# moritzmeister/hops-examples

Hardware: AMD Instinct MI355X
Metric: images/sec MNIST CNN + steps/sec Chicago-taxi DNN at 1/2/4/8 MI355X (higher is better)
Workload: dtype bf16; 1 GPU; model=MNIST CNN (experiment.mirrored model, 1394282 params), Adadelta(1.0), global_batch=32, per_gpu_batch=32, parallelism=dp1, engine=PersistentMnistStep, hipgraph=False, steps_per_execution=32, warmup_steps_run=5

## Files before the change

csrc/ops/bindings.cpp:

```cpp
#include <pybind11/pybind11.h>
#include <pybind11/stl.h>

#include <algorithm>
#include <memory>
#include <stdexcept>
#include <string>
#include <tuple>
#include <utility>
#include <vector>

#if defined(HOPSX_DEBUG) && HOPSX_DEBUG
#define HOPSX_DEBUG_BUILD 1
#else
#define HOPSX_DEBUG_BUILD 0
#endif

#include "ops_api.h"
extern "C" int hopsx_mnist_persist_occupancy(int dp);
extern "C" void hopsx_mnist_persist_reload_knobs();
extern "C" int hopsx_pad_cin(const float* w, long R, int C, int cp, float* out, void* out16, hipStream_t st);
extern "C" int hopsx_unpad_cin_add(float* gpad, long R, int C, int cp, float* tgt, hipStream_t st);

namespace py = pybind11;
extern "C" void hopsx_mlp_head_debug(void* p);
// ... 69 lines not shown
                      P<float>(arowsum), P<unsigned>(tickets), S(st));
  });
  m.def("conv2d_fwd", [](u x, u w, std::vector<int> g, int epi, u out, u bias, int act, u colsum, float xscale,
                         float xshift, u st) {
    return hopsx_conv2d_fwd(P<void>(x), P<void>(w), g.data(), epi, P<void>(out), P<float>(bias), act,
                            P<float>(colsum), xscale, xshift, S(st));
  });
  m.def("conv2d_fwd_res", [](u x, u w, std::vector<int> g, u out, u bias, int act, u residual, u st) {
    return hopsx_conv2d_fwd_res(P<void>(x), P<void>(w), g.data(), P<void>(out), P<float>(bias), act,
                                P<void>(residual), S(st));
  });
  m.def("conv2d_fwd_res_path", [](std::vector<int> g) { return hopsx_conv2d_fwd_res_path(g.data()); });
  m.def("conv2d_dgrad", [](u dy, u w, std::vector<int> g, u dx, u yprev, int act, u colsum, u y, int yact, u addend,
                           u st) {
    return hopsx_conv2d_dgrad(P<void>(dy), P<void>(w), g.data(), P<void>(dx), P<void>(yprev), act, P<float>(colsum),
                              P<void>(y), yact, P<void>(addend), S(st));
  });
  m.def("widedeep_slots", [](std::vector<long> iv, u out, long n) {
    return hopsx_widedeep_slots(iv.data(), (int)iv.size(), P<int>(out), n);
  });
  m.def("taxi_step2_ok", [](std::vector<long> iv, long rows) { return hopsx_taxi_step2_ok(iv.data(), (int)iv.size(), rows); });
  m.def("taxi_step2_xgeom", []() {
    std::vector<long> g(4);
    hopsx_taxi_step2_xgeom(g.data());
    return g;
  });
  m.def("taxi_step2", [](std::vector<uint64_t> p, std::vector<long> iv, std::vector<float> fv, long rows, u st) {
    return hopsx_taxi_step2(p.data(), (int)p.size(), iv.data(), (int)iv.size(), fv.data(), (int)fv.size(), rows, S(st));
  });
  def_arg_slots<true>(m, "taxi_step2", [](const ArgSlots& a, hipStream_t st) {
    return hopsx_taxi_step2(a.p.data(), (int)a.p.size(), a.iv.data(), (int)a.iv.size(), a.fv.data(), (int)a.fv.size(),
                            a.extra, st);
  });
  m.def("widedeep_step_lds", [](std::vector<long> iv) { return hopsx_widedeep_step_lds(iv.data(), (int)iv.size()); });
  m.def("set_deterministic", [](int on) {
    int e = 0;
#define X(tag) \
  if (!e) e = hopsx_det_set_##tag(on);
    HOPSX_DET_TUS(X)
#undef X
    return e;
  });
  m.attr("DEBUG") = HOPSX_DEBUG_BUILD;
  m.def("dbg_read", []() {
    static const std::pair<const char*, int (*)(unsigned*)> tus[] = {
#define X(tag) {#tag, hopsx_dbg_read_##tag},
        HOPSX_DBG_TUS(X)
#undef X
    };
    std::vector<std::tuple<std::string, unsigned, unsigned, unsigned, unsigned>> out;
    for (const auto& t : tus) {
      unsigned v[4] = {0u, 0u, 0u, 0u};
      const int e = t.second(v);
      if (e) throw std::runtime_error(std::string("hopsx dbg_read: hip error ") + std::to_string(e));
      if (v[0]) out.emplace_back(t.first, v[0], v[1], v[2], v[3]);
    }
    return out;
  });
  m.def("det_lost", []() {
    unsigned n = 0;
#define X(tag) n += hopsx_det_lost_##tag();
    HOPSX_DET_TUS(X)
#undef X
    return n;
  });
  m.def("mnist_persist", [](std::vector<uint64_t> p, std::vector<long> iv, std::vector<float> fv, u st) {
    return hopsx_mnist_persist(p.data(), (int)p.size(), iv.data(), (int)iv.size(), fv.data(), (int)fv.size(),
                               S(st));
  });
  def_arg_slots<false>(m, "mnist_persist", [](const ArgSlots& a, hipStream_t st) {
    return hopsx_mnist_persist(a.p.data(), (int)a.p.size(), a.iv.data(), (int)a.iv.size(), a.fv.data(),
                               (int)a.fv.size(), st);
  });
  m.def("mnist_eval", [](std::vector<uint64_t> p, std::vector<long> iv, std::vector<float> fv, u st) {
    return hopsx_mnist_eval(p.data(), (int)p.size(), iv.data(), (int)iv.size(), fv.data(), (int)fv.size(), S(st));
  });
  m.def("mnist_eval_tile", []() { return hopsx_mnist_eval_tile(); });
  m.def("taxi_eval", [](std::vector<uint64_t> p, std::vector<long> iv, u st) {
    return hopsx_taxi_eval(p.data(), (int)p.size(), iv.data(), (int)iv.size(), S(st));
  });
  m.def("taxi_eval_bins", []() { return hopsx_taxi_eval_bins(); });
  m.def("mnist_persist_reload_knobs", []() { hopsx_mnist_persist_reload_knobs(); });
  m.def("mnist_persist_occupancy", [](int dp) { return hopsx_mnist_persist_occupancy(dp); });
  m.def("pad_cin", [](u w, long R, int C, int cp, u out, u out16, u st) {
    return hopsx_pad_cin(P<float>(w), R, C, cp, P<float>(out), P<void>(out16), S(st));
  });
  m.def("unpad_cin_add", [](u g, long R, int C, int cp, u tgt, u st) {
    return hopsx_unpad_cin_add(P<float>(g), R, C, cp, P<float>(tgt), S(st));
  });
  m.def("mnist_persist_geom", []() {
    std::vector<long> g(24);
    hopsx_mnist_persist_geom(g.data());
    return g;
  });
  m.def("widedeep_step", [](std::vector<uint64_t> p, std::vector<long> iv, std::vector<float> fv, u st) {
    return hopsx_widedeep_step(p.data(), (int)p.size(), iv.data(), (int)iv.size(), fv.data(), (int)fv.size(),
                               S(st));
  });
  m.def("conv2d_fwd_pool_ok", [](std::vector<int> g, int act, int pk) { return hopsx_conv_fwd_pool_ok(g.data(), act, pk); });
  m.def("conv2d_fwd_pool", [](u x, u w, std::vector<int> g, u out, u am, u bias, int act, float p, u rng,
                              unsigned salt, int pk, u st) {
    return hopsx_conv2d_fwd_pool(P<void>(x), P<void>(w), g.data(), P<void>(out), P<void>(am), P<float>(bias), act, p,
                                 P<unsigned long long>(rng), salt, pk, S(st));
  });
  m.def("conv2d_fwd_pool_in_ok", [](std::vector<int> g0, std::vector<int> g, int act) {
    return hopsx_conv_fwd_pool_in_ok(g0.data(), g.data(), act);
  });
  m.def("conv2d_fwd_pool_in", [](u x0, float xscale, float xshift, u w0, u b0, int act0, std::vector<int> g0, u y1,
                                 u w, std::vector<int> g, u out, u am, u bias, int act, float p, u rng, unsigned salt,
                                 u st) {
    return hopsx_conv2d_fwd_pool_in(P<void>(x0), xscale, xshift, P<void>(w0), P<float>(b0), act0, g0.data(),
                                    P<void>(y1), P<void>(w), g.data(), P<void>(out), P<void>(am), P<float>(bias), act,
                                    p, P<unsigned long long>(rng), salt, S(st));
  });
  m.def("conv2d_dgrad_fused_wgrad_ok", [](std::vector<int> g, std::vector<int> g0) {
    return hopsx_conv_dgrad_fused_wgrad_ok(g.data(), g0.data());
  });
  m.def("conv2d_dgrad_fused_wgrad", [](u dy, u w, std::vector<int> g, u yprev, int act, u colsum, u y, int yact,
                                       std::vector<int> g0, u x0, float xscale, float xshift, u dw0, u st) {
    return hopsx_conv2d_dgrad_mfma_ex(P<void>(dy), P<void>(w), g.data(), nullptr, P<void>(yprev), act,
                                      P<float>(colsum), P<void>(y), yact, g0.data(), P<void>(x0), xscale, xshift,
                                      P<float>(dw0), S(st));
  });
  m.def("wgrad_debug_times", [](int n) {
    std::vector<unsigned long long> v((size_t)n);
    hopsx_wgrad_debug_times(v.data(), n);
    return v;
  });
  m.def("head_ce_ok", [](int C, int KD) { return hopsx_head_ce_ok(C, KD); });
  m.def("head_ce", [](int kind, u logits, int lf32, u target, int B, int C, int KD, float gs, u h, u w, u dw, u db,
                      u dh, u loss, u correct, u bias, u lout, float dp, u drng, unsigned dsalt, u st) {
    return hopsx_head_ce(kind, P<void>(logits), lf32, P<void>(target), B, C, KD, gs, P<void>(h), P<void>(w),
                         P<float>(dw), P<float>(db), P<void>(dh), P<float>(loss), P<int>(correct), P<float>(bias),
                         P<void>(lout), dp, P<unsigned long long>(drng), dsalt, S(st));
  });
  m.def("mlp_head_lds", [](int C, int N1) { return hopsx_mlp_head_lds(C, N1); });
  m.def("mlp_head_debug", [](u p) { hopsx_mlp_head_debug(P<void>(p)); });
  m.def("graph_upload", [](u exec, u st) {
    return (int)hipGraphUpload(reinterpret_cast<hipGraphExec_t>(exec), S(st));
  });
  m.def("mlp_head", [](u x, u w1, u b1, int act1, u y, u ws, u arrive, int B, int K, int N1, int kind, u target,
                       int C, float gs, u w2, u b2, u dw2, u db2, u dh, u loss, u correct, u lout, int lf32, float dp,
                       u drng, unsigned dsalt, u st) {
    return hopsx_mlp_head(P<void>(x), P<void>(w1), P<float>(b1), act1, P<void>(y), P<float>(ws), P<unsigned>(arrive),
                          B, K, N1, kind, P<void>(target), C, gs, P<void>(w2), P<float>(b2), P<float>(dw2),
                          P<float>(db2), P<void>(dh), P<float>(loss), P<int>(correct), P<void>(lout), lf32, dp,
                          P<unsigned long long>(drng), dsalt, S(st));
  });
  m.def("zero", [](u p, long bytes, u st) { return hopsx_zero(P<void>(p), bytes, S(st)); });
  m.def("nonfinite", [](u x, long n, int is_bf16, u out, u st) {
    return hopsx_nonfinite(P<void>(x), n, is_bf16, P<unsigned>(out), S(st));
  });
  m.def("linear_bwd_pair", [](u dy, u w, u x, u dx, u yprev, int act_prev, u colsum, u ay, int aact, u dw, u db,
                              int M, int N, int K, std::vector<int> pool, u pam, u px, u prng, unsigned psalt,
                              float pp, int dw_store, u st) {
    return hopsx_linear_bwd_pair(P<void>(dy), P<void>(w), P<void>(x), P<void>(dx), P<void>(yprev), act_prev,
                                 P<float>(colsum), P<void>(ay), aact, P<float>(dw), P<float>(db), M, N, K,
                                 pool.empty() ? nullptr : pool.data(), P<unsigned char>(pam), P<void>(px),
                                 P<unsigned long long>(prng), psalt, pp, dw_store, S(st));
  });
  m.def("conv2d_bwd_pair", [](u dy, u w, std::vector<int> g, u dx, u yprev, int act, u colsum, u y, int yact,
                              std::vector<int> g0, u x0, float xscale, float xshift, u dw0, u x, u dw, u db, u add,
                              u bnz, u bnmean, u bnrstd, u bnacc, u st) {
    return hopsx_conv2d_bwd_pair(P<void>(dy), P<void>(w), g.data(), P<void>(dx), P<void>(yprev), act,
                                 P<float>(colsum), P<void>(y), yact, g0.empty() ? nullptr : g0.data(), P<void>(x0),
                                 xscale, xshift, P<float>(dw0), P<void>(x), P<float>(dw), P<float>(db), P<void>(add),
// ... 186 lines not shown
```

csrc/ops/common.h:

```cpp
#pragma once
#include <hip/hip_runtime.h>
#include <stdint.h>

#define HOPSX_WAVE 64

typedef uint16_t bf16_raw;
typedef short bf16x8 __attribute__((ext_vector_type(8)));
typedef short bf16x4 __attribute__((ext_vector_type(4)));
typedef float f32x4 __attribute__((ext_vector_type(4)));

__device__ __forceinline__ bf16x8 zero_unless(bf16x8 v, bool keep) {
  const short m = keep ? (short)-1 : (short)0;
  return v & (bf16x8){m, m, m, m, m, m, m, m};
}
typedef __attribute__((address_space(3))) bf16x4* lds_v4_ptr;

__device__ __forceinline__ float bf2f(uint16_t v) { return __uint_as_float(((uint32_t)v) << 16); }

__device__ __forceinline__ uint16_t f2bf(float f) {
  uint32_t u = __float_as_uint(f);
  if ((u & 0x7fffffffu) > 0x7f800000u) return 0x7fc0;
  u += 0x7fffu + ((u >> 16) & 1u);
  return (uint16_t)(u >> 16);
}

__device__ __forceinline__ float wave_sum(float v) {
#pragma unroll
  for (int o = 32; o > 0; o >>= 1) v += __shfl_xor(v, o, 64);
  return v;
}
__device__ __forceinline__ float wave_max(float v) {
#pragma unroll
  for (int o = 32; o > 0; o >>= 1) v = fmaxf(v, __shfl_xor(v, o, 64));
  return v;
}

template <int R>
__device__ __forceinline__ float dpp_ror(float v) {
  return __builtin_bit_cast(float, __builtin_amdgcn_update_dpp(0, __builtin_bit_cast(int, v), 0x120 + R, 0xF, 0xF, false));
}
template <int CW>
__device__ __forceinline__ float row_fold(float v) {
  if constexpr (CW <= 1) v += dpp_ror<1>(v);
  if constexpr (CW <= 2) v += dpp_ror<2>(v);
  if constexpr (CW <= 4) v += dpp_ror<4>(v);
  if constexpr (CW <= 8) v += dpp_ror<8>(v);
  return v;
}

constexpr int kArriveWords = 9 * 32;
constexpr int HOPSX_BN_NREP = 8;
__device__ inline bool grid_arrive_last(unsigned* arrive) {
  const unsigned G = gridDim.x;
  const unsigned shard = blockIdx.x & 7u;
  const unsigned members = (G - shard + 7u) / 8u;
  unsigned* sw = arrive + 32u * (shard + 1u);
  if (atomicAdd(sw, 1u) != members - 1u) return false;
  atomicExch(sw, 0u);
  const unsigned shards = G < 8u ? G : 8u;
  if (atomicAdd(arrive, 1u) != shards - 1u) return false;
  atomicExch(arrive, 0u);
  return true;
}

__device__ __forceinline__ int xcd_remap(int bid, int nwg) {
  if (nwg <= 8) return bid;
  const int xcd = bid & 7, q = nwg >> 3, r = nwg & 7;
  const int base = (xcd < r) ? xcd * (q + 1) : r * (q + 1) + (xcd - r) * q;
  return base + (bid >> 3);
}

__device__ __forceinline__ uint32_t mix32(uint32_t x) {
  x ^= x >> 16;
  x *= 0x7feb352du;
  x ^= x >> 15;
  x *= 0x846ca68bu;
  x ^= x >> 16;
  return x;
}
__device__ __forceinline__ uint32_t hash_u32(uint64_t seed, uint64_t idx) {
  const uint32_t ka = (uint32_t)seed ^ (uint32_t)(idx >> 32) * 0x9E3779B9u;
  const uint32_t kb = (uint32_t)(seed >> 32);
  return mix32(mix32((uint32_t)idx ^ ka) + kb);
}
__device__ __forceinline__ float uniform01(uint64_t seed, uint64_t idx) {
  return (hash_u32(seed, idx) & 0xFFFFFF) * (1.0f / 16777216.0f);
}

__device__ __forceinline__ uint64_t drop_key(const unsigned long long* rng, unsigned salt) {
  return (uint64_t)rng[0] ^ ((uint64_t)salt * 0xD1B54A32D192ED03ull) ^ ((uint64_t)rng[1] * 0x8CB92BA72F3D8DD7ull);
}

enum Act : int { ACT_NONE = 0, ACT_RELU = 1, ACT_SIGMOID = 2, ACT_TANH = 3 };

__device__ __forceinline__ float apply_act(float v, int act) {
  switch (act) {
    case ACT_RELU: return v > 0.f ? v : 0.f;
    case ACT_SIGMOID: return 1.f / (1.f + __expf(-v));
    case ACT_TANH: return tanhf(v);
    default: return v;
  }
}
__device__ __forceinline__ float act_grad_from_out(float y, int act) {
  switch (act) {
    case ACT_RELU: return y > 0.f ? 1.f : 0.f;
    case ACT_SIGMOID: return y * (1.f - y);
    case ACT_TANH: return 1.f - y * y;
    default: return 1.f;
  }
}

#define HOPSX_CHECK_LAUNCH() (void)hipGetLastError()

#include <cstdlib>
#include <cstring>
static inline bool hopsx_disabled(const char* name) {
  const char* env = std::getenv("HOPSX_DISABLE");
  return env && *env && std::strstr(env, name) != nullptr;
}
static inline long hopsx_env_int(const char* name, long dflt) {
  const char* e = std::getenv(name);
  return e && *e ? std::atol(e) : dflt;
}

static inline bool hopsx_deterministic() {
  static const bool on = [] {
    const char* e = std::getenv("HOPSX_DETERMINISTIC");
    return e && *e == '1';
  }();
// ... 71 lines not shown
```

csrc/ops/mnist_persist.hip:

```cpp
#include "common.h"
#include "mnist_cnn.h"
#include "optim_core.h"
#include "wg_prims.h"

namespace mnistp {
using namespace wgp;
using namespace mnist_cnn;

constexpr int B = 32;
constexpr int NCONV = C2 * 128 + C2 + C1 * 4 + C1;
constexpr int OFF_B2 = C2 * 128, OFF_W1 = OFF_B2 + C2, OFF_B1 = OFF_W1 + C1 * 4;
constexpr int SLICE = 64, NSLICE = (NCONV + SLICE - 1) / SLICE;
constexpr int NRED = 19;
constexpr int NKC = (NPOS + NRED - 1) / NRED;
constexpr int NQ = SLICE / 4;
constexpr int NHEAD = B;
constexpr int GRID = NPOS + NHEAD;
constexpr int PAY = 272;
constexpr int PAY_DH = 0, PAY_H = 128, PAY_DL = 256, PAY_LOSS = 268, PAY_COR = 269;
constexpr int FL_A = 0, FL_B = 256, FL_C = 512, FL_D = 768, FL_WORDS = 1024;
constexpr int FL_EPOCH = FL_WORDS - 2;
constexpr int D_F32 = OFF_B2 * 2;
constexpr int D_BYTES = D_F32 + (NCONV - OFF_B2) * 4;
constexpr int TGB_N = NHEAD * (HID / 2);
constexpr int TG_WORDS = 2 * 2 * TGB_N;
static_assert(FL_WORDS % 2 == 0 && TGB_N % 256 == 0, "granules are 8-B aligned; every thread owns TGB_N / 256");
constexpr int HAND_FILL_C = 1 << 16;
constexpr int HAND_FILL_KEEP = 1 << 17;
constexpr int HAND_FMAX_SHIFT = 20;
constexpr int FCH = 4, NFCH = 32 / FCH;
static_assert(32 % FCH == 0 && NFCH <= 15, "whole chunks; the cap fits its 4 bits of Args::hand");

constexpr int DHS = row_stride(HID), DCS = row_stride(4 * B);
static_assert(DHS == 136 && DCS == 136, "strides the kernel was tuned with");

constexpr int L_W1 = 0;
constexpr int L_W2 = L_W1 + HID * W1S * 2;
constexpr int L_CW1 = L_W2 + C2 * W2S * 2;
constexpr int L_CB1 = L_CW1 + C1 * 4 * 4;
constexpr int L_CB2 = L_CB1 + C1 * 4;
constexpr int L_XIN = L_CB2 + C2 * 4;
constexpr int L_C1 = L_XIN + B * 16 * 4;
constexpr int L_POOL = L_C1 + B * 9 * C1S * 2;
constexpr int L_AM = L_POOL + B * PLS * 2;
constexpr int L_DH = L_AM + B * C2;
constexpr int L_DC2 = L_DH + B * DHS * 2;
constexpr int L_STG = L_DC2 + C2 * DCS * 2;
constexpr int L_RED = L_STG + NCONV * 4;
constexpr int L_SL = L_RED + NRED * SLICE * 4;
constexpr int L_KEEP = L_SL + 3 * 64 * 4;
constexpr int LDS_BYTES = L_KEEP + B * C2;

constexpr int H_W2 = 0;
constexpr int H_B2 = H_W2 + 3 * NCLS * HID * 4;
constexpr int H_B1 = H_B2 + 3 * 16 * 4;
constexpr int H_RED = H_B1 + 3 * HID * 4;
constexpr int H_H = H_RED + 8 * HID * 4;
constexpr int H_LOG = H_H + HID * 4;
constexpr int H_PAY = H_LOG + 16 * 4;
constexpr int H_ALL = H_PAY + PAY * 4;
constexpr int H_END = H_ALL + NHEAD * PAY * 4;
constexpr int H_DHS = H_END;
static_assert(H_DHS + B * DHS * 2 <= LDS_BYTES, "head LDS map must fit the position map");

constexpr int XMAX = 8;
constexpr long XS_POOL = (long)NPOS * 4 * 64 * 16;
constexpr long XS_DHT = 8L * 64 * 16;
constexpr int NFC2 = NCLS * HID + HID + NCLS, NFC2P = 1424;
constexpr long XS_FC2 = NFC2P * 4;
constexpr long XS_CONV = (long)NSLICE * SLICE * 4;
constexpr long XO_POOL = 0, XO_DHT = XO_POOL + 2L * XMAX * XS_POOL, XO_FC2 = XO_DHT + 2L * XMAX * XS_DHT,
               XO_CONV = XO_FC2 + 2L * XMAX * XS_FC2, X_BYTES = XO_CONV + 2L * XMAX * XS_CONV;
constexpr int XF_POOL = 0, XF_H = XMAX * NPOS, XF_CONV = XF_H + XMAX, XF_WORDS = XF_CONV + XMAX * NSLICE;
static_assert(NFC2 <= NFC2P && NFC2P % 4 == 0 && X_BYTES < 0x7fffffffL, "exchange geometry");
static_assert(LDS_BYTES <= 160 * 1024, "one workgroup per CU: 160 KiB LDS");
static_assert(L_RED + NRED * SLICE * 4 <= L_SL && 2 * 32 * 5 * 4 <= NRED * SLICE * 4, "reduce scratch");
static_assert(SLICE * 4 % 128 == 0 && NCONV * 4 % 128 == 0, "a slice row is whole 128-byte lines of an aligned slabC row");
static_assert(OFF_B2 % SLICE == 0 && D_F32 % 128 == 0 && D_BYTES % 128 == 0, "no slice straddles the bf16 / fp32 parts of D");
static_assert(NSLICE * SLICE >= NCONV && NSLICE <= NPOS && SLICE == 64, "slice geometry: one wave updates a slice");
static_assert(NQ == 16 && NRED > 16 && NRED - 16 <= 3 && 5 * NKC <= 64 && 2 * NKC <= 32 && NRED * (NKC - 1) < NPOS,
              "gather geometry: at most 5 groups' flags per wave, one per lane; both items' rows in one pend mask");

struct Args {
  float* master;
  bf16_raw* shadow;
  float* s1;
  float* s2;
  long off[8];
  const unsigned char* xs;
  const long long* ys;
  long nbatch;
  long long* cursor;
  unsigned long long* rng;
  float* step_dev;
  const float* hp_dev;
  float* slabA;
  float* slabB;
  float* slabC;
  float* slabD;
  unsigned* flags;
  unsigned* err;
  float* out;
  unsigned long long* dbg;
  OptHP hp;
  float drop_p, xscale, xshift;
  unsigned salt;
  int nsteps;
  int acquire;
  long long tmo;
  long long tmo0;
  int pollw, stagger;
  int pollw_a, pollw_b, pollw_c, pollw_d;
  int head1w;
  int hand;
  float inv_gb;
  int world, rank;
  int loopback;
  int xfence;
  long long* xstep;
  unsigned char* xbuf[XMAX];
  unsigned* xflag[XMAX];
};


__device__ __forceinline__ int xslot(const Args& a, int peer) { return a.loopback ? peer : a.rank; }

__device__ __forceinline__ bool wait_all(const unsigned* flags, int n, unsigned epoch, unsigned* err, unsigned code,
                                      int acquire, int* s_ok, long long tmo, int pollw = 1, int stagger = 0,
                                      int poll1 = 0) {
  if (pollw <= 1) {
    if (threadIdx.x < 64) {
      const int lane = threadIdx.x;
      int good = 1;
      const long long t0 = wall_clock64();
      for (unsigned spins = 0;; ++spins) {
        int ok = 1;
        unsigned e = poll1 ? flag_load(err) : 0u;
        for (int k = lane; k < n; k += 64) ok &= flag_load(flags + k) == epoch;
        if (__all(ok)) break;
        if (!poll1) e = flag_load(err);
        if (__builtin_amdgcn_readfirstlane(e) != 0u) {
          good = 0;
          break;
        }
        if ((spins & 15u) == 15u && wall_clock64() - t0 > tmo) {
          if (lane == 0) atomicCAS(err, 0u, code);
          good = 0;
          break;
        }
        __builtin_amdgcn_s_sleep(1);
      }
      if (acquire && good) __builtin_amdgcn_fence(__ATOMIC_ACQUIRE, "agent");
      drain();
      if (lane == 0) *s_ok = good;
    }
    __syncthreads();
    const int g = *s_ok;
    return g != 0;
  }
  volatile int* gen = s_ok + 1;
  const int wave = threadIdx.x >> 6;
  if (wave < pollw) {
    const int lane = threadIdx.x & 63;
    int good = 1;
    for (int d = 0; d < wave * stagger && __builtin_amdgcn_readfirstlane(*gen) != (int)code; ++d)
      __builtin_amdgcn_s_sleep(1);
    const long long t0 = wall_clock64();
    for (unsigned spins = 0;; ++spins) {
      if (__builtin_amdgcn_readfirstlane(*gen) == (int)code) break;
      int ok = 1;
      unsigned e = poll1 ? flag_load(err) : 0u;
      for (int k = lane; k < n; k += 64) ok &= flag_load(flags + k) == epoch;
      if (__all(ok)) {
        if (lane == 0) {
          s_ok[0] = 1;
          *gen = (int)code;
        }
        break;
      }
      if (!poll1) e = flag_load(err);
      if (__builtin_amdgcn_readfirstlane(e) != 0u) good = 0;
      if ((spins & 15u) == 15u && wall_clock64() - t0 > tmo) {
        if (lane == 0) atomicCAS(err, 0u, code);
        good = 0;
      }
      if (!good) {
        if (lane == 0) {
          s_ok[0] = 0;
          *gen = (int)code;
        }
        break;
      }
      __builtin_amdgcn_s_sleep(1);
    }
    if (acquire) __builtin_amdgcn_fence(__ATOMIC_ACQUIRE, "agent");
    drain();
  }
// ... 862 lines not shown
    for (int j = 0; j < 4; ++j)
#pragma unroll
      for (int r = 0; r < 4; ++r) {
        const int n = (2 * w + ii) * 16 + fq * 4 + r, co = j * 16 + fr;
        const long ai = a.off[4] + (long)n * KIN + p * C2 + co;
        a.master[ai] = wm[ii][j][r];
        a.s1[ai] = g1[ii][j][r];
        a.s2[ai] = g2[ii][j][r];
        a.shadow[ai] = f2bf_hw(wm[ii][j][r]);
      }
  if (owner && tid < SLICE) {
    const int e = p * SLICE + tid;
    if (e < NCONV) {
      const long ci = conv_idx(a, e);
      a.master[ci] = SLm[tid];
      a.s1[ci] = SL1[tid];
      a.s2[ci] = SL2[tid];
      a.shadow[ci] = f2bf_hw(SLm[tid]);
    }
  }
  stamp(a, a.nsteps - 1, 14);
  if (p == 0 && tid == 0) {
    if constexpr (DP) a.xstep[0] = xs0 + a.nsteps;
    a.cursor[0] = (cur0 + a.nsteps) % a.nbatch;
    *(unsigned long long*)(a.flags + FL_EPOCH) = eb + (unsigned long long)a.nsteps;
    a.rng[1] = ctr0 + (unsigned long long)a.nsteps;
    if (a.step_dev) a.step_dev[0] += (float)a.nsteps;
  }
}

template <bool DP>
__device__ __forceinline__ void head_wg(const Args& a, unsigned char* smem, int* s_ok, const OptHP& hp,
                                        long long cur0, long long xs0, unsigned long long eb) {
  const int i = blockIdx.x - NPOS;
  const int tid = threadIdx.x, lane = tid & 63;
  float* HW = (float*)(smem + H_W2);
  float* HW1 = HW + NCLS * HID;
  float* HW2 = HW1 + NCLS * HID;
  float* HB2 = (float*)(smem + H_B2);
  float* HB1 = (float*)(smem + H_B1);
  float* RED = (float*)(smem + H_RED);
  float* HH = (float*)(smem + H_H);
  float* LOG = (float*)(smem + H_LOG);
  float* PAYL = (float*)(smem + H_PAY);
  float* ALL = (float*)(smem + H_ALL);
  {
    constexpr int NJ = NCLS * HID / 256;
    float v0[NJ], v1[NJ], v2[NJ];
#pragma unroll
    for (int q = 0; q < NJ; ++q) {
      const long ai = a.off[6] + tid + 256 * q;
      v0[q] = a.master[ai];
      v1[q] = a.s1[ai];
      v2[q] = a.s2[ai];
    }
#pragma unroll
    for (int q = 0; q < NJ; ++q) {
      HW[tid + 256 * q] = v0[q];
      HW1[tid + 256 * q] = v1[q];
      HW2[tid + 256 * q] = v2[q];
    }
  }
  if (tid < NCLS) {
    const long ai = a.off[7] + tid;
    HB2[tid] = a.master[ai];
    HB2[16 + tid] = a.s1[ai];
    HB2[32 + tid] = a.s2[ai];
  }
  if (tid < HID) {
    const long ai = a.off[5] + tid;
    HB1[tid] = a.master[ai];
    HB1[128 + tid] = a.s1[ai];
    HB1[256 + tid] = a.s2[ai];
  }
  if (tid == 0) {
    PAYL[266] = PAYL[267] = PAYL[270] = PAYL[271] = 0.f;
  }
  __syncthreads();

  for (int s = 0; s < a.nsteps; ++s) {
    const unsigned ep = (unsigned)(eb + (unsigned long long)s + 1ull);
    const int par = s & 1;
    const int y = (int)a.ys[((cur0 + s) % a.nbatch) * B + i];
    if (!wait_all(a.flags + FL_A, NPOS, ep, a.err, s ? ecode(1, s) : ecode(12, 0), a.acquire, s_ok,
                  s ? a.tmo : a.tmo0, a.pollw_a, a.stagger, (a.hand & 2)))
      return;
    stamp(a, s, 0);
    {
      const int n4 = tid & 31, g = tid >> 5;
      const auto R = rsrc(a.slabA + (long)par * NPOS * B * HID);
      constexpr int NK = (NPOS + 7) / 8;
      f32x4 v[NK];
#pragma unroll
      for (int k = 0; k < NK; ++k) {
        const int pp = g + 8 * k;
        v[k] = pp < NPOS ? bld16<SC1>(R, ((pp * B + i) * HID + n4 * 4) * 4) : (f32x4){0.f, 0.f, 0.f, 0.f};
      }
      f32x4 acc = v[0];
#pragma unroll
      for (int k = 1; k < NK; ++k) acc += v[k];
      *(f32x4*)(RED + g * HID + n4 * 4) = acc;
    }
    __syncthreads();
    if (a.head1w) {
      if (tid < 64) {
        const int n0 = 2 * lane;
        float h[2];
#pragma unroll
        for (int u = 0; u < 2; ++u) {
          float v = 0.f;
#pragma unroll
          for (int g = 0; g < 8; ++g) v += RED[g * HID + n0 + u];
          h[u] = fmaxf(v + HB1[n0 + u], 0.f);
        }
        float z[NCLS];
#pragma unroll
        for (int c = 0; c < NCLS; ++c)
          z[c] = wave_sum(fmaf(h[1], HW[c * HID + n0 + 1], h[0] * HW[c * HID + n0])) + HB2[c];
        float m = z[0];
#pragma unroll
        for (int c = 1; c < NCLS; ++c) m = fmaxf(m, z[c]);
        float e[NCLS], se = 0.f, zy = 0.f;
        int am = NCLS;
#pragma unroll
        for (int c = NCLS - 1; c >= 0; --c) {
          e[c] = __expf(z[c] - m);
          if (z[c] == m) am = c;
          if (c == y) zy = z[c];
        }
#pragma unroll
        for (int c = 0; c < NCLS; ++c) se += e[c];
        const float inv_se = 1.f / se;
        float dl[NCLS];
#pragma unroll
        for (int c = 0; c < NCLS; ++c) dl[c] = (e[c] * inv_se - (c == y ? 1.f : 0.f)) * a.inv_gb;
        float dh[2];
#pragma unroll
        for (int u = 0; u < 2; ++u) {
          float d = 0.f;
#pragma unroll
          for (int c = 0; c < NCLS; ++c) d = fmaf(dl[c], HW[c * HID + n0 + u], d);
          dh[u] = h[u] > 0.f ? d : 0.f;
        }
        if (a.hand & 1)
          granule_store((unsigned long long*)(a.flags + FL_WORDS) + (par * NHEAD + i) * (HID / 2) + lane, ep,
                        (unsigned)f2bf_hw(dh[0]) | ((unsigned)f2bf_hw(dh[1]) << 16));
        const auto R = rsrc(a.slabB + ((long)par * NHEAD + i) * PAY);
        bst8<SC1>(R, (PAY_DH + n0) * 4, dh[0], dh[1]);
        bst8<SC1>(R, (PAY_H + n0) * 4, h[0], h[1]);
        float p0 = 0.f, p1 = 0.f;
#pragma unroll
        for (int c = 0; c < NCLS; c += 2)
          if (lane == c / 2) {
            p0 = dl[c];
            p1 = dl[c + 1];
          }
        if (lane < NCLS / 2) bst8<SC1>(R, (PAY_DL + 2 * lane) * 4, p0, p1);
        if (lane == NCLS / 2) bst8<SC1>(R, PAY_LOSS * 4, __logf(se) + m - zy, am == y ? 1.f : 0.f);
        drain();
        if (lane == 0) flag_store(a.flags + FL_B + i, ep);
      }
    }
    if (!a.head1w) {
    if (tid < HID) {
      float v = 0.f;
#pragma unroll
      for (int g = 0; g < 8; ++g) v += RED[g * HID + tid];
      HH[tid] = fmaxf(v + HB1[tid], 0.f);
    }
    __syncthreads();
    {
      const int c = tid >> 4, part = tid & 15;
      float v = 0.f;
      if (c < NCLS) {
#pragma unroll
        for (int k = 0; k < 8; ++k) v = fmaf(HH[part + 16 * k], HW[c * HID + part + 16 * k], v);
      }
      v = row_fold<1>(v);
      if (part == 0 && c < NCLS) LOG[c] = v + HB2[c];
    }
    __syncthreads();
    if (tid < 64) {
      const float z = lane < NCLS ? LOG[lane] : -INFINITY;
      const float m = wave_max(z);
      const float e = lane < NCLS ? __expf(z - m) : 0.f;
      const float se = wave_sum(e);
      const unsigned long long hit = __ballot(lane < NCLS && z == m);
      const int am = __ffsll((long long)hit) - 1;
      if (lane < NCLS) PAYL[PAY_DL + lane] = (e / se - (lane == y ? 1.f : 0.f)) * a.inv_gb;
      if (lane == 0) {
        PAYL[PAY_LOSS] = __logf(se) + m - LOG[y];
        PAYL[PAY_COR] = am == y ? 1.f : 0.f;
      }
    }
    __syncthreads();
    if (tid < HID) {
      const float h = HH[tid];
      float d = 0.f;
#pragma unroll
      for (int c = 0; c < NCLS; ++c) d = fmaf(PAYL[PAY_DL + c], HW[c * HID + tid], d);
      PAYL[PAY_DH + tid] = h > 0.f ? d : 0.f;
      PAYL[PAY_H + tid] = h;
    }
    __syncthreads();
    {
      if ((a.hand & 1) && tid < HID / 2)
        granule_store((unsigned long long*)(a.flags + FL_WORDS) + (par * NHEAD + i) * (HID / 2) + tid, ep,
                      (unsigned)f2bf_hw(PAYL[PAY_DH + 2 * tid]) | ((unsigned)f2bf_hw(PAYL[PAY_DH + 2 * tid + 1]) << 16));
      const auto R = rsrc(a.slabB + ((long)par * NHEAD + i) * PAY);
      if (tid < PAY / 4) bst16<SC1>(R, tid * 16, *(const f32x4*)(PAYL + tid * 4));
      drain();
      __syncthreads();
      if (tid == 0) flag_store(a.flags + FL_B + i, ep);
    }
    }
    stamp(a, s, 1);
    if (!wait_all(a.flags + FL_B, NHEAD, ep, a.err, s ? ecode(5, s) : ecode(12, 0), a.acquire, s_ok,
                  s ? a.tmo : a.tmo0, a.pollw, a.stagger, (a.hand & 2)))
      return;
    {
      const auto R = rsrc(a.slabB + (long)par * NHEAD * PAY);
      constexpr int NK = (NHEAD * PAY / 4 + 255) / 256;
      f32x4 v[NK];
#pragma unroll
// ... 108 lines not shown
      a.shadow[ai] = f2bf_hw(HW[j]);
    }
    if (tid < NCLS) {
      const long ai = a.off[7] + tid;
      a.master[ai] = HB2[tid];
      a.s1[ai] = HB2[16 + tid];
      a.s2[ai] = HB2[32 + tid];
      a.shadow[ai] = f2bf_hw(HB2[tid]);
    }
    if (tid < HID) {
      const long ai = a.off[5] + tid;
      a.master[ai] = HB1[tid];
      a.s1[ai] = HB1[128 + tid];
      a.s2[ai] = HB1[256 + tid];
      a.shadow[ai] = f2bf_hw(HB1[tid]);
    }
  }
}

template <bool DP>
__global__ __launch_bounds__(256, 1) void mnist_persist_k(const Args a) {
  extern __shared__ __attribute__((aligned(16))) unsigned char smem[];
  __shared__ int s_ok[3];
  stamp(a, 0, 13);
  if (threadIdx.x == 0) s_ok[0] = s_ok[1] = s_ok[2] = 0;
  const OptHP hp = load_hp(a.hp, a.hp_dev);
  const long long cur0 = a.cursor[0];
  const long long xs0 = DP ? a.xstep[0] : 0;
  const unsigned long long eb = *(const unsigned long long*)(a.flags + FL_EPOCH);
  if (blockIdx.x < NPOS) {
    position_wg<DP>(a, smem, s_ok, hp, cur0, a.rng[0], a.rng[1], xs0, eb);
  } else {
    head_wg<DP>(a, smem, s_ok, hp, cur0, xs0, eb);
  }
}

}

static int g_persist_reload = 0;
extern "C" void hopsx_mnist_persist_reload_knobs() { g_persist_reload = 1; }

extern "C" int hopsx_mnist_persist(const uint64_t* p, int np, const long* iv, int ni, const float* fv, int nf,
                                   hipStream_t st) {
  using namespace mnistp;
  if (np < 18 || ni < 18 || nf < 8) return (int)hipErrorInvalidValue;
  if (iv[11] != B || iv[10] < 1 || iv[8] < 1) return (int)hipErrorInvalidValue;
  const int world = (int)iv[13], rank = (int)iv[14];
  if (world < 1 || world > XMAX || rank < 0 || rank >= world) return (int)hipErrorInvalidValue;
  const bool dp = world > 1;
  if (dp && np < 19 + 2 * world) return (int)hipErrorInvalidValue;
  Args a{};
  a.master = (float*)p[0];
  a.shadow = (bf16_raw*)p[1];
  a.s1 = (float*)p[2];
  a.s2 = (float*)p[3];
  a.xs = (const unsigned char*)p[4];
  a.ys = (const long long*)p[5];
  a.cursor = (long long*)p[6];
  a.rng = (unsigned long long*)p[7];
  a.step_dev = (float*)p[8];
  a.hp_dev = (const float*)p[9];
  a.slabA = (float*)p[10];
  a.slabB = (float*)p[11];
  a.slabC = (float*)p[12];
  a.slabD = (float*)p[13];
  a.flags = (unsigned*)p[14];
  a.err = (unsigned*)p[15];
  a.out = (float*)p[16];
  a.dbg = (unsigned long long*)p[17];
  if (((uint64_t)a.slabC & 127) || ((uint64_t)a.slabD & 127)) return (int)hipErrorInvalidValue;
  for (int k = 0; k < 8; ++k) a.off[k] = iv[k];
  a.nbatch = iv[8];
  a.salt = (unsigned)iv[9];
  a.nsteps = (int)iv[10];
  a.acquire = (int)iv[12];
  a.world = world;
  a.rank = rank;
  a.loopback = (int)iv[15];
  a.xfence = (int)iv[17];
  a.tmo = (long long)iv[16] * 100000ll;
  a.tmo0 = a.tmo;
  static int kn_ok = 0, kn_pollw, kn_stagger, kn_a, kn_b, kn_c, kn_d, kn_head1w, kn_memset, kn_coop;
  static int kn_tagged, kn_gate, kn_poll1, kn_prog, kn_fill, kn_fmax;
  static long kn_start_ms;
  if (!kn_ok || g_persist_reload) {
    auto pw = [&](const char* name, long dflt) {
      const long v = hopsx_env_int(name, dflt);
      return (int)(v >= 1 && v <= 4 ? v : 1);
    };
    kn_pollw = pw("HOPSX_PERSIST_POLLW", 1);
    kn_stagger = (int)hopsx_env_int("HOPSX_PERSIST_STAGGER", 12);
    kn_a = pw("HOPSX_PERSIST_POLLW_A", kn_pollw);
    kn_b = pw("HOPSX_PERSIST_POLLW_B", kn_pollw);
    kn_c = pw("HOPSX_PERSIST_POLLW_C", 4);
    kn_d = pw("HOPSX_PERSIST_POLLW_D", kn_pollw);
    kn_head1w = (int)hopsx_env_int("HOPSX_PERSIST_HEAD1W", 1);
    kn_memset = (int)hopsx_env_int("HOPSX_PERSIST_MEMSET", 0);
    kn_coop = (int)hopsx_env_int("HOPSX_PERSIST_COOP", 0);
    kn_start_ms = hopsx_env_int("HOPSX_PERSIST_START_MS", 50);
    kn_tagged = hopsx_env_int("HOPSX_PERSIST_TAGGED", 1) != 0;
    const long gt = hopsx_env_int("HOPSX_PERSIST_GATE", NHEAD / 2);
    kn_gate = (int)(gt >= 1 && gt <= NHEAD ? gt : NHEAD / 2);
    kn_poll1 = hopsx_env_int("HOPSX_PERSIST_POLL1", 1) != 0;
    kn_prog = (int)(hopsx_env_int("HOPSX_PERSIST_PROG", 3) & 2);
    kn_fill = (int)(hopsx_env_int("HOPSX_PERSIST_FILL", 3) & 3);
    const long fm = hopsx_env_int("HOPSX_PERSIST_FILL_MAX", NFCH);
    kn_fmax = (int)(fm >= 0 && fm <= NFCH ? fm : NFCH);
    kn_ok = 1;
    g_persist_reload = 0;
  }
  a.pollw = kn_pollw;
  a.stagger = kn_stagger;
  a.pollw_a = kn_a;
  a.pollw_b = kn_b;
  a.pollw_c = kn_c;
  a.pollw_d = kn_d;
  a.head1w = kn_head1w;
  a.hand = kn_tagged | (kn_poll1 << 1) | (kn_prog << 2) | (kn_gate << 8) | (kn_fill << 16) | (kn_fmax << HAND_FMAX_SHIFT);
  if (kn_start_ms > 0 && kn_start_ms * 100000ll < a.tmo) a.tmo0 = kn_start_ms * 100000ll;
  a.inv_gb = 1.f / (float)(world * B);
  if (dp) {
    a.xstep = (long long*)p[18];
    for (int r = 0; r < world; ++r) {
      a.xbuf[r] = (unsigned char*)p[19 + r];
      a.xflag[r] = (unsigned*)p[19 + world + r];
      if (!a.xbuf[r] || !a.xflag[r] || ((uint64_t)a.xbuf[r] & 15)) return (int)hipErrorInvalidValue;
    }
  }
  a.drop_p = fv[0];
  a.xscale = fv[1];
  a.xshift = fv[2];
  a.hp = OptHP{fv[3], fv[4], fv[5], fv[6], fv[7], 0.f, 0.f, 0.f};
  static bool attr[2] = {false, false};
  const void* fn = dp ? (const void*)mnist_persist_k<true> : (const void*)mnist_persist_k<false>;
  if (!attr[dp]) {
    const hipError_t e = hipFuncSetAttribute(fn, hipFuncAttributeMaxDynamicSharedMemorySize, LDS_BYTES);
    if (e != hipSuccess) return (int)e;
    attr[dp] = true;
  }
  if (kn_memset) {
    const hipError_t e = hipMemsetAsync(a.flags, 0, FL_WORDS * sizeof(unsigned), st);
    if (e != hipSuccess) return (int)e;
  }
  if (kn_coop) {
    void* kargs[] = {(void*)&a};
    const hipError_t e = hipLaunchCooperativeKernel(fn, dim3(GRID), dim3(256), kargs, LDS_BYTES, st);
    if (e != hipSuccess) {
      (void)hipGetLastError();
      return (int)e;
    }
    return (int)hipSuccess;
  }
  if (dp)
    hipLaunchKernelGGL(mnist_persist_k<true>, dim3(GRID), dim3(256), LDS_BYTES, st, a);
  else
    hipLaunchKernelGGL(mnist_persist_k<false>, dim3(GRID), dim3(256), LDS_BYTES, st, a);
  return (int)hipGetLastError();
}

extern "C" int hopsx_mnist_persist_occupancy(int dp) {
  using namespace mnistp;
  const void* fn = dp ? (const void*)mnist_persist_k<true> : (const void*)mnist_persist_k<false>;
  if (hipFuncSetAttribute(fn, hipFuncAttributeMaxDynamicSharedMemorySize, LDS_BYTES) != hipSuccess) return -1;
  int n = 0;
  if (hipOccupancyMaxActiveBlocksPerMultiprocessor(&n, fn, 256, LDS_BYTES) != hipSuccess) return -1;
  return n;
}

extern "C" void hopsx_mnist_persist_geom(long* g) {
  using namespace mnistp;
  g[0] = B;
  g[1] = NPOS;
  g[2] = NHEAD;
  g[3] = GRID;
  g[4] = NCONV;
  g[5] = NSLICE;
  g[6] = SLICE;
  g[7] = PAY;
  g[8] = FL_WORDS;
  g[9] = LDS_BYTES;
  g[10] = D_BYTES;
  g[11] = X_BYTES;
  g[12] = XF_WORDS;
  g[13] = XMAX;
  g[14] = XO_POOL;
  g[15] = XS_POOL;
  g[16] = XO_DHT;
  g[17] = XS_DHT;
  g[18] = XO_FC2;
  g[19] = XS_FC2;
  g[20] = XO_CONV;
  g[21] = XS_CONV;
  g[22] = TG_WORDS;
  g[23] = NFCH;
}
```

csrc/ops/ops_api.h:

```cpp
#pragma once
#include <hip/hip_runtime.h>

enum GemmEpi : int { EPI_STORE_BF16 = 0, EPI_STORE_F32 = 1, EPI_ATOMIC_F32 = 2, EPI_DACT_BF16 = 3 };

extern "C" {
int hopsx_gemm(const void* A, long lda, int a_kc, const void* B, long ldb, int b_kc, int M, int N, int K, int epi,
               void* out, long ldo, const float* bias, float alpha, float beta, int act, const void* aux, long ldaux,
               float* colsum, float* ws, long ws_elems, const void* ay, int aact, float* arowsum, unsigned* tickets,
               hipStream_t st);
int hopsx_linear_bwd_pair(const void* dy, const void* w, const void* x, void* dx, const void* yprev, int act_prev,
                          float* colsum, const void* ay, int aact, float* dw, float* dbias, int M, int N, int K,
                          const int* pool, const unsigned char* pool_am, const void* pool_x,
                          const unsigned long long* pool_rng, unsigned pool_salt, float pool_p, int dw_store,
                          hipStream_t st);
int hopsx_conv2d_fwd(const void* x, const void* w, const int* geom, int epi, void* out, const float* bias, int act,
                     float* colsum, float xscale, float xshift, hipStream_t st);
int hopsx_conv2d_dgrad(const void* dy, const void* w, const int* geom, void* dx, const void* yprev, int act,
                       float* colsum, const void* y, int yact, const void* addend, hipStream_t st);
int hopsx_conv2d_wgrad(const void* dy, const void* x, const int* geom, float* dw, float* dbias, const void* y,
                       int yact, float* ws, long ws_elems, float xscale, float xshift, unsigned* counter,
                       hipStream_t st);

int hopsx_maxpool2d_fwd(const void* x, void* y, unsigned char* argmax, int B, int H, int W, int C, int OH, int OW,
                        int KH, int KW, int sh, int sw, int ph, int pw, float p, const unsigned long long* rng,
                        unsigned salt, hipStream_t st);
int hopsx_maxpool2d_bwd(const void* dy, const unsigned char* argmax, const void* x, void* dx, int B, int H, int W,
                        int C, int OH, int OW, int KH, int KW, int sh, int sw, int ph, int pw, int act,
                        float* colsum, float p, const unsigned long long* rng, unsigned salt, hipStream_t st);
int hopsx_maxpool2d_fwd_path(const void* x, const void* y, const unsigned char* argmax, int B, int H, int W, int C,
                             int OH, int OW, int KH, int KW, int sh, int sw, int ph, int pw);
int hopsx_maxpool2d_bwd_path(const void* dy, const unsigned char* argmax, const void* x, const void* dx, int B, int H,
                             int W, int C, int OH, int OW, int KH, int KW, int sh, int sw, int ph, int pw,
                             int has_colsum);
int hopsx_avgpool_global_fwd(const void* x, void* y, int B, int HW, int C, hipStream_t st);
int hopsx_avgpool_global_bwd(const void* dy, void* dx, int B, int HW, int C, hipStream_t st);

bool hopsx_head_ce_ok(int C, int KD);
int hopsx_head_ce(int kind, const void* logits, int logits_f32, const void* target, int B, int C, int KD,
                  float grad_scale, const void* h, const void* w, float* dw, float* db, void* dh, float* loss_sum,
                  int* correct, const float* bias, void* logits_out, float drop_p,
                  const unsigned long long* drop_rng, unsigned drop_salt, hipStream_t st);
int hopsx_mlp_head_lds(int C, int N1);
int hopsx_mlp_head(const void* x, const void* w1, const float* b1, int act1, void* y, float* ws, unsigned* arrive,
                   int B, int K, int N1, int kind, const void* target, int C, float grad_scale, const void* w2,
                   const float* b2, float* dw2, float* db2, void* dh, float* loss_sum, int* correct,
                   void* logits_out, int logits_f32, float drop_p, const unsigned long long* drop_rng,
                   unsigned drop_salt, hipStream_t st);
int hopsx_loss_fwd_bwd(int kind, const void* logits, int logits_f32, const void* target, int B, int C,
                       float grad_scale, float* loss_sum, int* correct, void* dlogits, int dlogits_f32,
                       hipStream_t st);

int hopsx_optim_step(int kind, float* param, float* grad, float* s1, float* s2, float* s3, void* shadow_bf16,
                     long n, const float* hp, int nhp, float* step_dev, unsigned* arrive, unsigned long long* rng,
                     int zero_grad, const void* const* pf_src, void* const* pf_dst, const long* pf_bytes,
                     int pf_njobs, long long* pf_cursor, int pf_nbatch, const float* hp_dev, hipStream_t st);

int hopsx_dropout_fwd(const void* x, void* y, long n, float p, const unsigned long long* rng, unsigned salt,
                      hipStream_t st);
int hopsx_dropout_bwd(const void* dy, void* dx, long n, float p, const unsigned long long* rng, unsigned salt,
                      hipStream_t st);
int hopsx_rng_advance(unsigned long long* rng, hipStream_t st);

int hopsx_cast_f32_bf16(const float* x, void* y, long n, hipStream_t st);
int hopsx_cast_bf16_f32(const void* x, float* y, long n, hipStream_t st);
int hopsx_u8_normalize(const unsigned char* x, void* y, long n, float scale, float shift, hipStream_t st);
int hopsx_colsum_bf16(const void* x, float* out, int M, int N, hipStream_t st);
int hopsx_act_bwd(const void* dy, const void* y, void* dx, long n, int act, hipStream_t st);
int hopsx_act_bwd_colsum(const void* dy, const void* y, void* dx, int M, int N, int act, float* colsum,
                         hipStream_t st);
int hopsx_add_bf16(const void* a, const void* b, void* out, long n, int act, hipStream_t st);

int hopsx_bn_fwd_train(const void* x, void* y, const float* gamma, const float* beta, float* mean_out,
                       float* rstd_out, float* running_mean, float* running_var, float momentum, float eps, int M,
                       int C, const void* residual, int act, float* acc, hipStream_t st);
int hopsx_bn_fwd_infer(const void* x, void* y, const float* gamma, const float* beta, const float* running_mean,
                       const float* running_var, float eps, int M, int C, const void* residual, int act,
                       hipStream_t st);
int hopsx_bn_bwd(const void* dy, const void* x, const void* y, const float* gamma, const float* mean,
                 const float* rstd, void* dx, float* dgamma, float* dbeta, float* ws, int M, int C, int act,
                 void* dresidual, float* acc, const float* zbeta, hipStream_t st);

long hopsx_widedeep_step_lds(const long* iv, int ni);
int hopsx_widedeep_slots(const long* iv, int ni, int* out, long n);
int hopsx_widedeep_step(const uint64_t* ptrs, int np, const long* iv, int ni, const float* fv, int nf,
                        hipStream_t st);
long hopsx_taxi_step2_ok(const long* iv, int ni, long rows);
void hopsx_taxi_step2_xgeom(long* g);
int hopsx_taxi_step2(const uint64_t* ptrs, int np, const long* iv, int ni, const float* fv, int nf, long rows,
                     hipStream_t st);
int hopsx_mnist_persist(const uint64_t* ptrs, int np, const long* iv, int ni, const float* fv, int nf,
                        hipStream_t st);
void hopsx_mnist_persist_geom(long* g);
int hopsx_mnist_eval(const uint64_t* ptrs, int np, const long* iv, int ni, const float* fv, int nf, hipStream_t st);
int hopsx_mnist_eval_tile();
int hopsx_taxi_eval(const uint64_t* ptrs, int np, const long* iv, int ni, hipStream_t st);
int hopsx_taxi_eval_bins();

bool hopsx_conv_fwd_mfma_ok(const int* geom);
bool hopsx_conv_fwd_pool_ok(const int* geom, int act, int pk);
bool hopsx_conv_fwd_pool_in_ok(const int* geom0, const int* geom, int act);
int hopsx_conv2d_fwd_pool_in(const void* x0, float xscale, float xshift, const void* w0, const float* b0, int act0,
                             const int* geom0, void* y1, const void* w, const int* geom, void* out, void* am,
                             const float* bias, int act, float p, const unsigned long long* rng, unsigned salt,
                             hipStream_t st);
int hopsx_conv2d_fwd_pool(const void* x, const void* w, const int* geom, void* out, void* am, const float* bias, int act,
                          float p, const unsigned long long* rng, unsigned salt, int pk, hipStream_t st);
bool hopsx_conv_dgrad_mfma_ok(const int* geom);
int hopsx_conv2d_fwd_mfma(const void* x, const void* w, const int* geom, void* out, const float* bias, int act,
                          hipStream_t st);
int hopsx_conv2d_fwd_mfma_ex(const void* x, const void* w, const int* geom, void* out, const float* bias, int act,
                             float* bnacc, hipStream_t st);
int hopsx_conv2d_fwd_res(const void* x, const void* w, const int* geom, void* out, const float* bias, int act,
                         const void* residual, hipStream_t st);
int hopsx_conv2d_fwd_res_path(const int* geom);
int hopsx_conv2d_fwd_mfma_res(const void* x, const void* w, const int* geom, void* out, const float* bias, int act,
                              const void* res, hipStream_t st);
int hopsx_conv2d_fwd_bnstats(const void* x, const void* w, const int* geom, void* out, float* bnacc, hipStream_t st);
int hopsx_conv2d_fwd_bnstats_inbn(const void* z, void* a, const void* w, const int* geom, void* out, float* bnacc,
                                  float* inacc, const float* gamma, const float* beta, float* mean_out,
                                  float* rstd_out, float* rmean, float* rvar, float momentum, float eps, int act,
                                  hipStream_t st);
int hopsx_conv2d_fwd_mfma_inbn(const void* z, void* a, const void* w, const int* geom, void* out, float* bnacc,
                               float* inacc, const float* gamma, const float* beta, float* mean_out, float* rstd_out,
                               float* rmean, float* rvar, float momentum, float eps, int act, hipStream_t st);
int hopsx_bn_fwd_apply_fin(const void* x, void* y, const float* gamma, const float* beta, float* mean_out,
                           float* rstd_out, float* running_mean, float* running_var, float momentum, float eps, int M,
                           int C, const void* residual, int act, float* acc, hipStream_t st);
int hopsx_bn_prestats_ok(int C);
int hopsx_bn_coop_timeouts(const float* acc, int C);
int hopsx_conv2d_dgrad_mfma(const void* dy, const void* w, const int* geom, void* dx, const void* yprev,
                            int act_prev, float* colsum, const void* y, int yact, hipStream_t st);
bool hopsx_conv_wgrad_mfma_ok(const int* geom);
int hopsx_conv2d_bwd_pair(const void* dy, const void* w, const int* geom, void* dx, const void* yprev, int act_prev,
                          float* colsum, const void* y, int yact, const int* geom0, const void* x0, float xscale,
                          float xshift, float* dw0, const void* x, float* dw, float* dbias, const void* addend,
                          const void* bnz, const float* bnmean, const float* bnrstd, float* bnacc, hipStream_t st);
int hopsx_conv2d_dgrad_bn(const void* dy, const void* w, const int* geom, void* dx, const void* yprev, int act_prev,
                          const void* addend, const void* bnz, const float* bnmean, const float* bnrstd, float* bnacc,
                          hipStream_t st);
int hopsx_conv2d_dgrad_mfma_bn(const void* dy, const void* w, const int* geom, void* dx, const void* yprev,
                               int act_prev, const void* addend, const void* bnz, const float* bnmean,
                               const float* bnrstd, float* bnacc, hipStream_t st);
int hopsx_conv2d_bwd_pair_bn_ok(const int* geom);
int hopsx_bn_bwd_pre(const void* dy, const void* x, const float* gamma, const float* mean, const float* rstd,
                     void* dx, float* dgamma, float* dbeta, float* ws, int M, int C, float* acc, hipStream_t st);
int hopsx_wgrad_debug_times(unsigned long long* host_out, int n);
int hopsx_conv_wgrad_glds_ok(const int* geom);
int hopsx_conv2d_wgrad_glds(const void* dy, const void* x, const int* geom, float* dw, int force, hipStream_t st);
int hopsx_conv2d_wgrad_mfma(const void* dy, const void* x, const int* geom, float* dw, float* dbias, const void* y,
                            int yact, hipStream_t st);
bool hopsx_conv_dgrad_fused_wgrad_ok(const int* geom, const int* geom0);
int hopsx_conv2d_dgrad_mfma_ex(const void* dy, const void* w, const int* geom, void* dx, const void* yprev,
                               int act_prev, float* colsum, const void* y, int yact, const int* geom0,
                               const void* x0, float xscale, float xshift, float* dw0, hipStream_t st);

int hopsx_zero(void* p, long bytes, hipStream_t st);
int hopsx_nonfinite(const void* x, long n, int is_bf16, unsigned* out, hipStream_t st);

int hopsx_embedding_bag_fwd(const float* table, const long* idx, const long* offsets, int nbags, int dim,
                            long nidx, int bag_len, int mode, void* out, int out_f32, long ldo, long rows,
                            hipStream_t st);
int hopsx_embedding_bag_bwd(const void* dout, int dout_f32, long ldo, const long* idx, const long* offsets,
                            int nbags, int dim, long nidx, int bag_len, int mode, float* dtable, long rows,
                            hipStream_t st);

int hopsx_column_stats(const float* x, int rows, int cols, float* out_stats, hipStream_t st);
int hopsx_column_hist(const float* x, int rows, int cols, const float* mins, const float* maxs, int bins,
                      unsigned* hist, hipStream_t st);
int hopsx_gram(const float* x, const float* mean, int rows, int cols, float* gram, hipStream_t st);

int hopsx_taxi_transform(const float* raw, const int* vids, long n, const int* ints, const float* flts,
                         const long* offs, float* dense, long* cat, float* label, hipStream_t st);
int hopsx_transform_max_bounds();

int hopsx_prefix_sum_f64(const double* v, long n, double* P, double* work, hipStream_t st);
// ... 9 lines not shown
```

Baseline: 1.518 million images/sec.

## Preload head operands, add permlane wave-sum tree, and gate A-flag polling

In the persistent MNIST step, the head's bias and weight operands are loaded into registers before the wait on stage-A flags, which takes global loads off the critical path after the barrier. A new wave reduction uses v_permlane32/16_swap plus DPP rotates in place of the shuffle-based wave_sum. A lane-parallel pre-poll gate with sleep and a tick timeout runs before the existing wait_all. All three are on by default through env knobs, and a probe kernel is added to check the tree sum against the reference. The tree sum may give slightly different float rounding, and the preloaded operands add register pressure.

```diff
diff --git a/csrc/ops/bindings.cpp b/csrc/ops/bindings.cpp
--- a/csrc/ops/bindings.cpp
+++ b/csrc/ops/bindings.cpp
@@ -175,6 +175,9 @@
   m.def("taxi_eval_bins", []() { return hopsx_taxi_eval_bins(); });
   m.def("mnist_persist_reload_knobs", []() { hopsx_mnist_persist_reload_knobs(); });
   m.def("mnist_persist_occupancy", [](int dp) { return hopsx_mnist_persist_occupancy(dp); });
+  m.def("wave_sum_probe", [](u x, long rows, u out_ref, u out_tree, u st) {
+    return hopsx_wave_sum_probe(P<float>(x), rows, P<float>(out_ref), P<float>(out_tree), S(st));
+  });
   m.def("pad_cin", [](u w, long R, int C, int cp, u out, u out16, u st) {
     return hopsx_pad_cin(P<float>(w), R, C, cp, P<float>(out), P<void>(out16), S(st));
   });
diff --git a/csrc/ops/common.h b/csrc/ops/common.h
--- a/csrc/ops/common.h
+++ b/csrc/ops/common.h
@@ -45,6 +45,20 @@
   if constexpr (CW <= 2) v += dpp_ror<2>(v);
   if constexpr (CW <= 4) v += dpp_ror<4>(v);
   if constexpr (CW <= 8) v += dpp_ror<8>(v);
+  return v;
+}
+
+__device__ __forceinline__ float wave_sum_tree(float v) {
+  float a0 = v, a1 = v;
+  asm volatile("s_nop 1\n\tv_permlane32_swap_b32 %0, %1\n\ts_nop 0" : "+v"(a0), "+v"(a1));
+  v = a0 + a1;
+  float b0 = v, b1 = v;
+  asm volatile("s_nop 1\n\tv_permlane16_swap_b32 %0, %1\n\ts_nop 0" : "+v"(b0), "+v"(b1));
+  v = b0 + b1;
+  v += dpp_ror<8>(v);
+  v += dpp_ror<4>(v);
+  v += dpp_ror<2>(v);
+  v += dpp_ror<1>(v);
   return v;
 }
 
diff --git a/csrc/ops/mnist_persist.hip b/csrc/ops/mnist_persist.hip
--- a/csrc/ops/mnist_persist.hip
+++ b/csrc/ops/mnist_persist.hip
@@ -28,6 +28,10 @@
 constexpr int HAND_FILL_C = 1 << 16;
 constexpr int HAND_FILL_KEEP = 1 << 17;
 constexpr int HAND_FMAX_SHIFT = 20;
+constexpr int HAND_GATEA_SHIFT = 18;
+constexpr int HAND_HEAD_REGS = 1 << 24;
+constexpr int HAND_HEAD_TREE = 1 << 25;
+constexpr int NLINE_A = (NPOS + 31) / 32;
 constexpr int FCH = 4, NFCH = 32 / FCH;
 static_assert(32 % FCH == 0 && NFCH <= 15, "whole chunks; the cap fits its 4 bits of Args::hand");
 
@@ -113,6 +117,7 @@
   int pollw_a, pollw_b, pollw_c, pollw_d;
   int head1w;
   int hand;
+  int gate_a_tk;
   float inv_gb;
   int world, rank;
   int loopback;
@@ -1141,6 +1146,33 @@
     const unsigned ep = (unsigned)(eb + (unsigned long long)s + 1ull);
     const int par = s & 1;
     const int y = (int)a.ys[((cur0 + s) % a.nbatch) * B + i];
+    float rb1[2], rw[NCLS][2], rb2[NCLS];
+    auto head_operands = [&]() {
+      const int n0 = 2 * lane;
+#pragma unroll
+      for (int u = 0; u < 2; ++u) rb1[u] = HB1[n0 + u];
+#pragma unroll
+      for (int c = 0; c < NCLS; ++c) {
+#pragma unroll
+        for (int u = 0; u < 2; ++u) rw[c][u] = HW[c * HID + n0 + u];
+        rb2[c] = HB2[c];
+      }
+#pragma unroll
+      for (int u = 0; u < 2; ++u) asm volatile("" : "+v"(rb1[u]));
+#pragma unroll
+      for (int c = 0; c < NCLS; ++c) asm volatile("" : "+v"(rw[c][0]), "+v"(rw[c][1]), "+v"(rb2[c]));
+    };
+    if (tid < 64 && a.head1w && (a.hand & HAND_HEAD_REGS)) head_operands();
+    if (const int ga = (a.hand >> HAND_GATEA_SHIFT) & 3; ga && tid < 64) {
+      const int l0 = ga == 1 ? (i % NLINE_A) * 32 : 0;
+      const bool mine = lane < 32 && l0 + lane < NPOS;
+      const long long t0 = wall_clock64();
+      for (;;) {
+        const unsigned f = mine ? flag_load(a.flags + FL_A + l0 + lane) : ep;
+        if (__all(f == ep) || wall_clock64() - t0 >= a.gate_a_tk) break;
+        __builtin_amdgcn_s_sleep(4);
+      }
+    }
     if (!wait_all(a.flags + FL_A, NPOS, ep, a.err, s ? ecode(1, s) : ecode(12, 0), a.acquire, s_ok,
                   s ? a.tmo : a.tmo0, a.pollw_a, a.stagger, (a.hand & 2)))
       return;
@@ -1164,18 +1196,23 @@
     if (a.head1w) {
       if (tid < 64) {
         const int n0 = 2 * lane;
+        if (!(a.hand & HAND_HEAD_REGS)) head_operands();
         float h[2];
 #pragma unroll
         for (int u = 0; u < 2; ++u) {
           float v = 0.f;
 #pragma unroll
           for (int g = 0; g < 8; ++g) v += RED[g * HID + n0 + u];
-          h[u] = fmaxf(v + HB1[n0 + u], 0.f);
+          h[u] = fmaxf(v + rb1[u], 0.f);
         }
         float z[NCLS];
-#pragma unroll
-        for (int c = 0; c < NCLS; ++c)
-          z[c] = wave_sum(fmaf(h[1], HW[c * HID + n0 + 1], h[0] * HW[c * HID + n0])) + HB2[c];
+        if (a.hand & HAND_HEAD_TREE) {
+#pragma unroll
+          for (int c = 0; c < NCLS; ++c) z[c] = wave_sum_tree(fmaf(h[1], rw[c][1], h[0] * rw[c][0])) + rb2[c];
+        } else {
+#pragma unroll
+          for (int c = 0; c < NCLS; ++c) z[c] = wave_sum(fmaf(h[1], rw[c][1], h[0] * rw[c][0])) + rb2[c];
+        }
         float m = z[0];
 #pragma unroll
         for (int c = 1; c < NCLS; ++c) m = fmaxf(m, z[c]);
@@ -1198,7 +1235,7 @@
         for (int u = 0; u < 2; ++u) {
           float d = 0.f;
 #pragma unroll
-          for (int c = 0; c < NCLS; ++c) d = fmaf(dl[c], HW[c * HID + n0 + u], d);
+          for (int c = 0; c < NCLS; ++c) d = fmaf(dl[c], rw[c][u], d);
           dh[u] = h[u] > 0.f ? d : 0.f;
         }
         if (a.hand & 1)
@@ -1473,6 +1510,7 @@
   a.tmo0 = a.tmo;
   static int kn_ok = 0, kn_pollw, kn_stagger, kn_a, kn_b, kn_c, kn_d, kn_head1w, kn_memset, kn_coop;
   static int kn_tagged, kn_gate, kn_poll1, kn_prog, kn_fill, kn_fmax;
+  static int kn_gate_a, kn_gate_a_tk, kn_head;
   static long kn_start_ms;
   if (!kn_ok || g_persist_reload) {
     auto pw = [&](const char* name, long dflt) {
@@ -1497,6 +1535,11 @@
     kn_fill = (int)(hopsx_env_int("HOPSX_PERSIST_FILL", 3) & 3);
     const long fm = hopsx_env_int("HOPSX_PERSIST_FILL_MAX", NFCH);
     kn_fmax = (int)(fm >= 0 && fm <= NFCH ? fm : NFCH);
+    const long ga = hopsx_env_int("HOPSX_PERSIST_GATE_A", 1);
+    kn_gate_a = (int)(ga >= 0 && ga <= 2 ? ga : 0);
+    const long gus = hopsx_env_int("HOPSX_PERSIST_GATE_A_US", 20);
+    kn_gate_a_tk = (int)(gus >= 0 && gus <= 1000000 ? gus * 100 : 2000);
+    kn_head = (int)(hopsx_env_int("HOPSX_PERSIST_HEAD_CHAIN", 3) & 3);
     kn_ok = 1;
     g_persist_reload = 0;
   }
@@ -1507,7 +1550,9 @@
   a.pollw_c = kn_c;
   a.pollw_d = kn_d;
   a.head1w = kn_head1w;
-  a.hand = kn_tagged | (kn_poll1 << 1) | (kn_prog << 2) | (kn_gate << 8) | (kn_fill << 16) | (kn_fmax << HAND_FMAX_SHIFT);
+  a.hand = kn_tagged | (kn_poll1 << 1) | (kn_prog << 2) | (kn_gate << 8) | (kn_fill << 16) | (kn_fmax << HAND_FMAX_SHIFT) |
+           (kn_gate_a << HAND_GATEA_SHIFT) | (kn_head & 1 ? HAND_HEAD_REGS : 0) | (kn_head & 2 ? HAND_HEAD_TREE : 0);
+  a.gate_a_tk = kn_gate_a_tk;
   if (kn_start_ms > 0 && kn_start_ms * 100000ll < a.tmo) a.tmo0 = kn_start_ms * 100000ll;
   a.inv_gb = 1.f / (float)(world * B);
   if (dp) {
@@ -1585,3 +1630,15 @@
   g[22] = TG_WORDS;
   g[23] = NFCH;
 }
+
+__global__ __launch_bounds__(64) void wave_sum_probe_k(const float* x, float* out_ref, float* out_tree) {
+  const long e = (long)blockIdx.x * 64 + threadIdx.x;
+  const float v = x[e];
+  out_ref[e] = wave_sum(v);
+  out_tree[e] = wave_sum_tree(v);
+}
+extern "C" int hopsx_wave_sum_probe(const float* x, long rows, float* out_ref, float* out_tree, hipStream_t st) {
+  if (rows < 1 || rows > 65535 || !x || !out_ref || !out_tree) return (int)hipErrorInvalidValue;
+  hipLaunchKernelGGL(wave_sum_probe_k, dim3((unsigned)rows), dim3(64), 0, st, x, out_ref, out_tree);
+  return (int)hipGetLastError();
+}
diff --git a/csrc/ops/ops_api.h b/csrc/ops/ops_api.h
--- a/csrc/ops/ops_api.h
+++ b/csrc/ops/ops_api.h
@@ -91,6 +91,7 @@
 int hopsx_mnist_persist(const uint64_t* ptrs, int np, const long* iv, int ni, const float* fv, int nf,
                         hipStream_t st);
 void hopsx_mnist_persist_geom(long* g);
+int hopsx_wave_sum_probe(const float* x, long rows, float* out_ref, float* out_tree, hipStream_t st);
 int hopsx_mnist_eval(const uint64_t* ptrs, int np, const long* iv, int ni, const float* fv, int nf, hipStream_t st);
 int hopsx_mnist_eval_tile();
 int hopsx_taxi_eval(const uint64_t* ptrs, int np, const long* iv, int ni, hipStream_t st);
```

New measurement: 1.551 million images/sec (median of 6 runs). +2.2%, better.
